# refresh-bio/colord

Hardware: AMD Instinct MI355X
Metric: input Gbases/s + archive size vs ref, ONT 50 Gb at 1/2/4/8 MI355X (higher is better)
Workload: dtype u64

## Files before the change

### colord_amd/csrc/anchors.hip

```cpp
#include "common.hpp"
#include "objects.hpp"
#include <algorithm>

struct cl_anchors {
	cl_ctx* ctx = nullptr;
	uint32_t n_reads = 0, c = 0;
	uint64_t n_anchors = 0;
	DevBuf<uint32_t> n_cands;
	DevBuf<uint32_t> cand;
	DevBuf<uint64_t> cand_off;
	DevBuf<uint32_t> anchors;
};

namespace {

struct Arena { const uint64_t* packed; const uint64_t* word_off; const uint32_t* lens; };

__device__ inline uint64_t mmer_at(const Arena& A, uint64_t wb, uint32_t p, uint32_t m)
{
	const uint64_t* w = A.packed + wb + (p >> 5);
	const uint32_t j = p & 31;
	const uint64_t hi = w[0], lo = w[1];
	const uint32_t s = 128 - 2 * (j + m);
	const uint64_t v = (s >= 64) ? (hi >> (s - 64)) : ((hi << (64 - s)) | (lo >> s));
	return v & ((1ULL << (2 * m)) - 1);
}
__device__ inline uint64_t mmer_of(uint64_t hi, uint64_t lo, uint32_t p, uint32_t m)
{
	const uint32_t s = 128 - 2 * ((p & 31) + m);
	const uint64_t v = (s >= 64) ? (hi >> (s - 64)) : ((hi << (64 - s)) | (lo >> s));
	return v & ((1ULL << (2 * m)) - 1);
}
__device__ inline uint64_t revcomp_m(uint64_t x, uint32_t m)
{
	x = ~x; x = __brevll(x);
	x = ((x >> 1) & 0x5555555555555555ULL) | ((x & 0x5555555555555555ULL) << 1);
	return x >> (64 - 2 * m);
}
__device__ inline uint64_t ref_mmer(const Arena& R, uint32_t id, bool rev, uint32_t q, uint32_t m)
{
	const uint32_t len = R.lens[id];
	const uint64_t wb = R.word_off[id];
	return rev ? revcomp_m(mmer_at(R, wb, len - m - q, m), m) : mmer_at(R, wb, q, m);
}

struct BuildSlot { uint64_t key; uint32_t head; uint32_t strands; };
typedef uint2 EncSlot;
constexpr uint32_t LINK_POS = 0x3fffffffu;
__device__ inline uint32_t tag_of(uint64_t hash) { return (uint32_t)((hash * 0xD6E8FEB86659FD93ULL) >> 32); }
__device__ inline uint32_t table_slot(uint64_t hash, uint32_t tsz) { return (uint32_t)(((uint64_t)(uint32_t)(hash >> 17) * tsz) >> 32); }
struct EncTable { EncSlot* slots; const uint64_t* toff; uint32_t* next; const uint64_t* noff; };
constexpr uint32_t REGION_SLOTS = 2048;
constexpr uint64_t KEY_EMPTY = ~0ULL;
constexpr uint32_t NIL = 0xffffffffu;

__global__ void k_table_sizes(const uint32_t* __restrict__ lens, const uint8_t* __restrict__ has_n, const uint32_t* __restrict__ ncand,
                              uint32_t r0, uint32_t r1, uint32_t m, uint32_t x4, uint32_t lds_max_n, uint32_t* __restrict__ tsize, uint32_t* __restrict__ nsize, uint32_t* __restrict__ err)
{
	uint32_t r = r0 + blockIdx.x * blockDim.x + threadIdx.x;
	if (r >= r1) return;
	uint32_t len = lens[r];
	bool active = ncand[r] > 0 && !has_n[r] && len >= m;
	uint32_t n = active ? len - m + 1 : 0;
	if (n <= lds_max_n) n = 0;
	uint32_t t = 0;
	if (n) { t = 16; while (t < 2 * n + n / 2 && t < REGION_SLOTS) t <<= 1; if (t >= REGION_SLOTS) t = (uint32_t)(((uint64_t)n * x4 / 4 + REGION_SLOTS - 1) / REGION_SLOTS * REGION_SLOTS); }
	tsize[r - r0] = t; nsize[r - r0] = n;
}
constexpr uint32_t REGION = REGION_SLOTS, INS_T = 256;
__global__ __launch_bounds__(INS_T) void k_table_insert(Arena A, uint32_t r0, uint32_t r1, uint32_t m, EncTable T, uint32_t* __restrict__ n_distinct,
                                                       uint2* __restrict__ bins , uint32_t* __restrict__ err)
{
	__shared__ BuildSlot reg[REGION];
	__shared__ uint32_t cnt[512], start[513];
	const uint32_t r = r0 + blockIdx.x;
	if (r >= r1) return;
	const uint64_t t0 = T.toff[r - r0]; const uint32_t tsz = (uint32_t)(T.toff[r - r0 + 1] - t0);
	if (!tsz) return;
	const uint64_t n0 = T.noff[r - r0]; const uint32_t n = (uint32_t)(T.noff[r - r0 + 1] - n0);
	const uint64_t wb = A.word_off[r];
	const uint32_t lane = threadIdx.x & 63;
	const uint32_t rs = tsz < REGION ? tsz : REGION, n_reg = tsz / rs, rshift = 31 - (uint32_t)__clz((int)rs);
	uint2* bin = bins + n0;
	uint32_t fresh = 0;
	for (uint32_t rg0 = 0; rg0 < n_reg; rg0 += 512)
	{
		const uint32_t nr = n_reg - rg0 < 512 ? n_reg - rg0 : 512;
		for (uint32_t i = threadIdx.x; i < 512; i += INS_T) cnt[i] = 0;
		__syncthreads();
		for (uint32_t p = threadIdx.x; p < n; p += INS_T)
		{
			const uint64_t xf = mmer_at(A, wb, p, m), xr = revcomp_m(xf, m), x = xf < xr ? xf : xr;
			const uint32_t h = table_slot(hash_mm(x), tsz), rg = (h >> rshift) - rg0;
			if (rg < nr) atomicAdd(&cnt[rg], 1u);
		}
		__syncthreads();
		if (threadIdx.x == 0) { uint32_t a = 0; for (uint32_t i = 0; i < nr; ++i) { start[i] = a; a += cnt[i]; cnt[i] = 0; } start[nr] = a; }
		__syncthreads();
		for (uint32_t p = threadIdx.x; p < n; p += INS_T)
		{
			const uint64_t xf = mmer_at(A, wb, p, m), xr = revcomp_m(xf, m), x = xf < xr ? xf : xr;
			const uint32_t h = table_slot(hash_mm(x), tsz), rg = (h >> rshift) - rg0;
			if (rg < nr) bin[start[rg] + atomicAdd(&cnt[rg], 1u)] = make_uint2(p, h);
		}
		__syncthreads();
		__threadfence_block();
		for (uint32_t rg = 0; rg < nr; ++rg)
		{
			for (uint32_t i = threadIdx.x; i < rs; i += INS_T) { reg[i].key = KEY_EMPTY; reg[i].head = NIL; reg[i].strands = 0; }
			__syncthreads();
			const uint32_t b = start[rg], e = start[rg + 1];
			for (uint32_t i = b + threadIdx.x; i < e; i += INS_T)
			{
				const uint2 ph = bin[i];
				const uint32_t pp = ph.x;
				const uint64_t xf = mmer_at(A, wb, pp, m), xr = revcomp_m(xf, m), x = xf < xr ? xf : xr;
				uint32_t off = ph.y & (rs - 1), tries = 0;
				for (;;)
				{
					unsigned long long old = atomicCAS((unsigned long long*)&reg[off].key, (unsigned long long)KEY_EMPTY, (unsigned long long)x);
					if (old == KEY_EMPTY || old == x) break;
					off = (off + 1) & (rs - 1);
					if (++tries > rs) { atomicOr(err, 2u); break; }
				}
				const uint32_t strand = xf != x ? 1u : 0u;
				T.next[n0 + pp] = atomicExch(&reg[off].head, pp | (strand << 31));
				if (!(atomicOr(&reg[off].strands, 1u << strand) & (1u << strand))) ++fresh;
			}
			__syncthreads();
			EncSlot* dst = T.slots + t0 + (uint64_t)(rg0 + rg) * rs;
			for (uint32_t i = threadIdx.x; i < rs; i += INS_T) dst[i] = make_uint2(reg[i].head == NIL ? 0u : tag_of(hash_mm(reg[i].key)), reg[i].head);
			__syncthreads();
		}
	}
	fresh = wave_sum(fresh);
	if (lane == 0 && fresh) atomicAdd(&n_distinct[r - r0], fresh);
}
struct TaskCfg { uint32_t r0, r1, c, m; uint32_t pe, pr; double frac_always, frac_min, max_mult; };

constexpr uint32_t FILT_WORDS = 2048, STAGE = 128;
__device__ inline uint32_t filt_word(uint64_t hash) { return (uint32_t)(hash >> 46) & (FILT_WORDS - 1); }
__device__ inline uint64_t filt_mask(uint64_t hash) { return (1ull << ((hash >> 40) & 63)) | (1ull << ((hash >> 34) & 63)) | (1ull << ((hash >> 28) & 63)); }
__device__ __host__ inline uint32_t match_segments(uint32_t n, uint32_t seg_n) { return (seg_n == 0 || n <= seg_n + seg_n / 2) ? 1u : (n + seg_n - 1) / seg_n; }
__global__ __launch_bounds__(256) void k_match(Arena A, Arena R, EncTable T, TaskCfg cfg, const uint32_t* __restrict__ cand_refs, const uint32_t* __restrict__ cand_n,
                                              const uint32_t* __restrict__ n_distinct, const uint2* __restrict__ work , uint32_t n_work, uint32_t seg_n,
                                              unsigned long long* __restrict__ n_pairs, uint64_t cap, uint64_t* __restrict__ pairs)
{
	__shared__ unsigned long long filt[FILT_WORDS];
	__shared__ uint64_t stage_all[4][STAGE];
	if (blockIdx.x >= n_work) return;
	const uint32_t rl = work[blockIdx.x].x, seg = work[blockIdx.x].y;
	const uint32_t lane = threadIdx.x & 63, wv = threadIdx.x >> 6;
	const uint32_t r = cfg.r0 + rl;
	const uint64_t t0 = T.toff[rl]; const uint32_t tsz = (uint32_t)(T.toff[rl + 1] - t0);
	const uint32_t n_slots = cand_n[r] < cfg.c ? cand_n[r] : cfg.c;
	if (tsz == 0 || n_slots == 0) return;
	const uint32_t elen = A.lens[r];
	if ((double)n_distinct[rl] < cfg.frac_min * (double)elen && !((double)n_distinct[rl] > cfg.frac_always * (double)elen)) return;
	for (uint32_t i = threadIdx.x; i < FILT_WORDS; i += 256) filt[i] = 0;
	__syncthreads();
	uint32_t p_lo, p_hi;
	{
		const uint64_t ewb = A.word_off[r]; const uint32_t n = elen - cfg.m + 1;
		const uint32_t nseg = match_segments(n, seg_n);
		if (seg >= nseg) return;
		p_lo = (uint32_t)((uint64_t)n * seg / nseg); p_hi = (uint32_t)((uint64_t)n * (seg + 1) / nseg);
		for (uint32_t p = p_lo + threadIdx.x; p < p_hi; p += 256)
		{
			const uint64_t xf = mmer_at(A, ewb, p, cfg.m), xr = revcomp_m(xf, cfg.m);
			const uint64_t hash = hash_mm(xf < xr ? xf : xr);
			atomicOr(&filt[filt_word(hash)], (unsigned long long)filt_mask(hash));
		}
	}
	__syncthreads();
	const uint64_t n0 = T.noff[rl];
	const uint64_t ewb = A.word_off[r];
	uint64_t* stage = stage_all[wv]; uint32_t fill = 0;
	auto flush = [&]() {
		if (!fill) return;
		unsigned long long base = 0;
		if (lane == 0) base = atomicAdd(n_pairs, (unsigned long long)fill);
		base = ((unsigned long long)__shfl((int)(base >> 32), 0, 64) << 32) | (uint32_t)__shfl((int)(uint32_t)base, 0, 64);
		if (base + fill <= cap) for (uint32_t i = lane; i < fill; i += 64) pairs[base + i] = stage[i];
		fill = 0;
	};
	for (uint32_t slot = 0; slot < n_slots; ++slot)
	{
		const uint32_t id = cand_refs[(uint64_t)r * cfg.c + slot], rlen = R.lens[id];
		if (rlen < cfg.m) continue;
		const uint64_t rwb = R.word_off[id];
		const uint32_t nq = rlen - cfg.m + 1, sl = rl * cfg.c + slot;
		const uint32_t PR = cfg.pr; const uint32_t pr_mask = (1u << PR) - 1;
		const uint64_t key_rev = (uint64_t)(2 * sl) << (cfg.pe + PR), key_fwd = (uint64_t)(2 * sl + 1) << (cfg.pe + PR);
		if (threadIdx.x == 0 && seg == 0) atomicAdd(n_pairs + 1, (unsigned long long)nq);
		const uint64_t* rw = R.packed + rwb;
		struct Probe { uint64_t x; uint2 slot; uint32_t h, tag; bool pass, fwd_other, rev_other; };
		auto probe = [&](uint32_t q, uint64_t hi, uint64_t lo) -> Probe
		{
			Probe P{ 0, make_uint2(0u, NIL), 0, 0, false, false, false };
			if (q < nq)
			{
				const uint64_t y = mmer_of(hi, lo, q, cfg.m), z = revcomp_m(y, cfg.m), x = y < z ? y : z;
				const uint64_t hash = hash_mm(x);
				const uint64_t fm = filt_mask(hash);
				if ((filt[filt_word(hash)] & fm) == fm)
				{
					P.pass = true; P.x = x; P.fwd_other = y != x; P.rev_other = z != x;
					P.h = table_slot(hash, tsz); P.tag = tag_of(hash);
					P.slot = T.slots[t0 + P.h];
				}
			}
			return P;
		};
		uint64_t hi1 = 0, lo1 = 0, hi2 = 0, lo2 = 0;
		Probe cur;
		{
			const uint32_t q = wv * 64 + lane;
			uint64_t hi = 0, lo = 0;
			if (q < nq) { hi = rw[q >> 5]; lo = rw[(q >> 5) + 1]; }
			if (q + 256 < nq) { hi1 = rw[(q + 256) >> 5]; lo1 = rw[((q + 256) >> 5) + 1]; }
			cur = probe(q, hi, lo);
		}
		const uint32_t rmask = (tsz < REGION ? tsz : REGION) - 1;
		for (uint32_t q0 = wv * 64; q0 < nq; q0 += 256)
		{
			const uint32_t q = q0 + lane;
			hi2 = 0; lo2 = 0;
			if (q + 512 < nq) { hi2 = rw[(q + 512) >> 5]; lo2 = rw[((q + 512) >> 5) + 1]; }
			const Probe nxt = probe(q + 256, hi1, lo1);
			uint32_t head = NIL, cnt = 0;
			const uint32_t fs = cur.fwd_other ? 1u : 0u, rs_ = cur.rev_other ? 1u : 0u;
			if (cur.pass)
			{
				uint2 sl8 = cur.slot; uint32_t h = cur.h;
				while (sl8.y != NIL)
				{
					if (sl8.x == cur.tag)
					{
						const uint64_t xf = mmer_at(A, ewb, sl8.y & LINK_POS, cfg.m), xr = revcomp_m(xf, cfg.m);
						if ((xf < xr ? xf : xr) == cur.x) { head = sl8.y; break; }
					}
					h = (h & ~rmask) | ((h + 1) & rmask);
					sl8 = T.slots[t0 + h];
				}
				for (uint32_t p = head; p != NIL; p = T.next[n0 + (p & LINK_POS)])
					if ((p & LINK_POS) >= p_lo && (p & LINK_POS) < p_hi) cnt += (uint32_t)((p >> 31) == fs) + (uint32_t)((p >> 31) == rs_);
			}
			cur = nxt; hi1 = hi2; lo1 = lo2;
			if (!__any(cnt != 0)) continue;
			const uint32_t incl = wave_incl_scan(cnt), tot = __shfl(incl, 63, 64);
			const uint64_t kf = key_fwd | (uint64_t)(~q & pr_mask), kr = key_rev | (uint64_t)(~(nq - 1 - q) & pr_mask);
			if (fill + tot > STAGE) flush();
			if (tot <= STAGE)
			{
				uint32_t o = fill + incl - cnt;
				for (uint32_t p = head; p != NIL; p = T.next[n0 + (p & LINK_POS)])
				{
					if ((p & LINK_POS) < p_lo || (p & LINK_POS) >= p_hi) continue;
					const uint64_t pos = (uint64_t)(p & LINK_POS) << PR;
					if ((p >> 31) == fs) stage[o++] = kf | pos;
					if ((p >> 31) == rs_) stage[o++] = kr | pos;
				}
				fill += tot;
				continue;
			}
			unsigned long long base = 0;
			if (lane == 0) base = atomicAdd(n_pairs, (unsigned long long)tot);
			base = ((unsigned long long)__shfl((int)(base >> 32), 0, 64) << 32) | (uint32_t)__shfl((int)(uint32_t)base, 0, 64);
			if (base + tot > cap) continue;
			uint64_t o = base + incl - cnt;
			for (uint32_t p = head; p != NIL; p = T.next[n0 + (p & LINK_POS)])
			{
				if ((p & LINK_POS) < p_lo || (p & LINK_POS) >= p_hi) continue;
				const uint64_t pos = (uint64_t)(p & LINK_POS) << PR;
				if ((p >> 31) == fs) pairs[o++] = kf | pos;
				if ((p >> 31) == rs_) pairs[o++] = kr | pos;
			}
		}
	}
	flush();
}
template<uint32_t MAXN> struct LdsGeom { static constexpr uint32_t SLOTS = ((MAXN + MAXN / 2) + 17) & ~1u, WORDS = (MAXN + 27 + 31) / 32 + 2; };
__device__ inline uint32_t lds_table_slots(uint32_t n) { const uint32_t s = (n + n / 2 + 1) & ~1u; return s < 16 ? 16 : s; }
template<uint32_t MAXN, uint32_t FW, uint32_t NT, uint32_t WAVES_PER_SIMD>
__global__ __launch_bounds__(NT, WAVES_PER_SIMD) void k_match_lds(Arena A, Arena R, TaskCfg cfg, uint32_t min_n, const uint8_t* __restrict__ has_n,
                                                 const uint32_t* __restrict__ cand_refs, const uint32_t* __restrict__ cand_n, uint32_t* __restrict__ n_distinct, uint32_t n_reads,
                                                 unsigned long long* __restrict__ n_pairs, uint64_t cap, uint64_t* __restrict__ pairs, uint32_t dbg)
{
	static_assert(MAXN <= 65535 && (FW & (FW - 1)) == 0 && NT % 64 == 0, "positions are 16-bit links; 0xffff is the empty slot");
	constexpr uint32_t NW = NT / 64, LSTAGE = 64;
	__shared__ unsigned long long filt[FW];
	__shared__ uint64_t rd[LdsGeom<MAXN>::WORDS];
	__shared__ uint32_t slots32[LdsGeom<MAXN>::SLOTS / 2];
	__shared__ uint64_t stage_all[NW][LSTAGE];
	__shared__ uint32_t s_distinct;
	const uint32_t rl = blockIdx.x;
	if (rl >= n_reads) return;
	const uint32_t r = cfg.r0 + rl, m = cfg.m;
	const uint32_t elen = A.lens[r];
	const uint32_t n_slots = cand_n[r] < cfg.c ? cand_n[r] : cfg.c;
	if (n_slots == 0 || has_n[r] || elen < m) return;
	const uint32_t n = elen - m + 1;
	if (n <= min_n || n > MAXN) return;
	const uint32_t lane = threadIdx.x & 63, wv = threadIdx.x >> 6;
	const uint32_t S = lds_table_slots(n);
	const uint16_t* slot16 = (const uint16_t*)slots32;
	{
		const uint64_t* src = A.packed + A.word_off[r];
		const uint32_t nw = (elen + 31) / 32 + 1;
		for (uint32_t i = threadIdx.x; i < nw; i += NT) rd[i] = src[i];
		for (uint32_t i = threadIdx.x; i < FW; i += NT) filt[i] = 0;
		for (uint32_t i = threadIdx.x; i < S / 2; i += NT) slots32[i] = 0xffffffffu;
		if (threadIdx.x == 0) s_distinct = 0;
	}
	__syncthreads();
	if (dbg == 1) return;
	auto own = [&](uint32_t p) -> uint64_t { return mmer_of(rd[p >> 5], rd[(p >> 5) + 1], p, m); };
	auto step = [&](uint32_t off) -> uint32_t { return off + 1 == S ? 0u : off + 1; };
	{
		uint32_t fresh = 0;
		for (uint32_t p = threadIdx.x; p < n; p += NT)
		{
			const uint64_t xf = own(p), xr = revcomp_m(xf, m), hash = hash_mm(xf < xr ? xf : xr);
			atomicOr(&filt[(uint32_t)(hash >> 46) & (FW - 1)], (unsigned long long)filt_mask(hash));
			bool dup = false;
			for (uint32_t off = table_slot(hash, S);;)
			{
				uint32_t* w = &slots32[off >> 1]; const uint32_t sh = (off & 1) * 16;
				const uint32_t old = *(volatile uint32_t*)w, q = (old >> sh) & 0xffffu;
				if (q != 0xffffu) { if (!dup && own(q) == xf) dup = true; off = step(off); continue; }
				if (atomicCAS(w, old, (old & ~(0xffffu << sh)) | (p << sh)) == old) break;
			}
			fresh += dup ? 0u : 1u;
		}
		fresh = wave_sum(fresh);
		if (lane == 0 && fresh) atomicAdd(&s_distinct, fresh);
	}
	__syncthreads();
	const uint32_t nd = s_distinct;
	if (threadIdx.x == 0) n_distinct[rl] = nd;
	if (dbg == 2) return;
	if ((double)nd < cfg.frac_min * (double)elen && !((double)nd > cfg.frac_always * (double)elen)) return;
	uint64_t* stage = stage_all[wv]; uint32_t fill = 0;
	auto flush = [&]() {
		if (!fill) return;
		unsigned long long base = 0;
		if (lane == 0) base = atomicAdd(n_pairs, (unsigned long long)fill);
		base = ((unsigned long long)__shfl((int)(base >> 32), 0, 64) << 32) | (uint32_t)__shfl((int)(uint32_t)base, 0, 64);
		if (base + fill <= cap) for (uint32_t i = lane; i < fill; i += 64) pairs[base + i] = stage[i];
		fill = 0;
	};
	struct Look { uint64_t y, z; uint32_t h0, cnt, nh, hp0, hp1, hf0, hf1; };
	auto look = [&](bool live, uint32_t q, uint64_t hi, uint64_t lo) -> Look {
		Look L{ 0, 0, 0, 0, 0, 0, 0, 0, 0 };
		if (!live) return L;
// ... 372 lines not shown
		if (i < n)
		{
			const uint32_t t = sel_task[i] & 0x7fffffffu, slot = (t / 2) % c;
			o_cand[4 * s] = cand_refs[(uint64_t)r * c + slot]; o_cand[4 * s + 1] = (t & 1) == 0 ? 1u : 0u;
			o_cand[4 * s + 2] = sel_tot[i]; o_cand[4 * s + 3] = sel_n[i];
			o_task[(uint64_t)rl * c + i] = sel_task[i]; o_count[(uint64_t)rl * c + i] = sel_n[i];
		}
		else { o_cand[4 * s] = ~0u; o_cand[4 * s + 1] = 0; o_cand[4 * s + 2] = 0; o_cand[4 * s + 3] = 0; o_task[(uint64_t)rl * c + i] = ~0u; o_count[(uint64_t)rl * c + i] = 0; }
	}
}
__global__ void k_copy_fix(const uint32_t* __restrict__ o_task, const uint64_t* __restrict__ slot_off, uint64_t n_slots,
                           const uint64_t* __restrict__ pair_off, const uint32_t* __restrict__ anch, uint64_t dst_base, uint32_t* __restrict__ out,
                           TaskCfg cfg, const uint32_t* __restrict__ kanch, const uint64_t* __restrict__ common_off, uint64_t common_base)
{
	const uint64_t s = (uint64_t)blockIdx.x * blockDim.x + threadIdx.x;
	if (s >= n_slots) return;
	const uint32_t tm = o_task[s];
	if (tm == ~0u) return;
	const uint32_t t = tm & 0x7fffffffu;
	const uint32_t n = (uint32_t)(slot_off[s + 1] - slot_off[s]);
	const uint32_t* src = anch + 3 * pair_off[t];
	if (tm & 0x80000000u)
	{
		const uint64_t gs = (uint64_t)cfg.r0 * cfg.c + t / 2;
		const uint64_t o = common_off[gs] - common_base; const uint32_t nk = (uint32_t)(common_off[gs + 1] - common_off[gs]);
		src = kanch + 6 * o + (uint64_t)(t & 1) * 3 * nk;
	}
	uint32_t* dst = out + 3 * (dst_base + slot_off[s]);
	for (uint32_t i = 0; i < 3 * n; ++i) dst[i] = src[i];
	for (uint32_t i = 0; i + 1 < n; ++i)
	{
		const uint32_t end = dst[3 * i + 2] + dst[3 * i];
		if (dst[3 * (i + 1) + 2] < end) { const uint32_t d = end - dst[3 * (i + 1) + 2]; dst[3 * (i + 1) + 2] += d; dst[3 * (i + 1)] -= d; dst[3 * (i + 1) + 1] += d; }
	}
	for (uint32_t i = 0; i + 1 < n; ++i)
	{
		const uint32_t end = dst[3 * i + 1] + dst[3 * i];
		if (dst[3 * (i + 1) + 1] < end) { const uint32_t d = end - dst[3 * (i + 1) + 1]; dst[3 * (i + 1) + 1] += d; dst[3 * (i + 1)] -= d; dst[3 * (i + 1) + 2] += d; }
	}
}
__global__ void k_add_u64(uint64_t* v, uint64_t n, uint64_t c) { uint64_t i = (uint64_t)blockIdx.x * blockDim.x + threadIdx.x; if (i < n) v[i] += c; }
}

extern "C" cl_status cl_anchor_candidates_hifi(cl_ctx* ctx, const cl_reads* reads, const cl_reads* refs, const uint32_t* d_cand_refs, const uint32_t* d_cand_n,
                                               uint32_t c, uint32_t anchor_len, double frac_always, double frac_min, double max_matches_mult,
                                               uint32_t min_anchors, uint32_t kmer_len, uint32_t modulo, const uint64_t* d_common_off, const uint64_t* d_common, cl_anchors** out);
extern "C" cl_status cl_anchor_candidates(cl_ctx* ctx, const cl_reads* reads, const cl_reads* refs, const uint32_t* d_cand_refs, const uint32_t* d_cand_n,
                                          uint32_t c, uint32_t anchor_len, double frac_always, double frac_min, double max_matches_mult,
                                          uint32_t min_anchors, cl_anchors** out)
{
	return cl_anchor_candidates_hifi(ctx, reads, refs, d_cand_refs, d_cand_n, c, anchor_len, frac_always, frac_min, max_matches_mult, min_anchors, 0, 0, nullptr, nullptr, out);
}
extern "C" cl_status cl_anchor_candidates_hifi(cl_ctx* ctx, const cl_reads* reads, const cl_reads* refs, const uint32_t* d_cand_refs, const uint32_t* d_cand_n,
                                               uint32_t c, uint32_t anchor_len, double frac_always, double frac_min, double max_matches_mult,
                                               uint32_t min_anchors, uint32_t kmer_len, uint32_t modulo, const uint64_t* d_common_off, const uint64_t* d_common, cl_anchors** out)
{
	if (!ctx || !reads || !refs || !d_cand_refs || !d_cand_n || !out) return cl_fail(ctx, CL_E_INVALID, "cl_anchor_candidates: null argument");
	const bool hifi = d_common_off != nullptr;
	if (hifi && (kmer_len < 2 || kmer_len > 28 || modulo == 0)) return cl_fail(ctx, CL_E_INVALID, "cl_anchor_candidates_hifi: 2 <= kmer_len <= 28, modulo >= 1");
	if (c == 0 || c > 16 || anchor_len < 2 || anchor_len > 28) return cl_fail(ctx, CL_E_INVALID, "cl_anchor_candidates: 1 <= c <= 16, 2 <= anchor_len <= 28");
	HIP_TRY(ctx, hipSetDevice(ctx->device));
	const uint32_t nr = reads->n_reads, m = anchor_len;
	cl_anchors* X = new cl_anchors(); X->ctx = ctx; X->n_reads = nr; X->c = c;
	std::unique_ptr<cl_anchors> guard(X);
	DEV_ALLOC(ctx, X->n_cands, nr); DEV_ALLOC(ctx, X->cand, (uint64_t)nr * c * 4); DEV_ALLOC(ctx, X->cand_off, (uint64_t)nr * c + 1);
	Arena A{ reads->packed.p, reads->word_off.p, reads->lens.p }, R{ refs->packed.p, refs->word_off.p, refs->lens.p };
	std::vector<uint32_t> h_len(nr);
	if (nr) HIP_TRY(ctx, hipMemcpy(h_len.data(), reads->lens.p, (uint64_t)nr * 4, hipMemcpyDeviceToHost));
	auto bits_for = [](uint64_t v) -> uint32_t { uint32_t b = 1; while ((1ull << b) <= v) ++b; return b; };
	uint32_t max_ref_len = 0;
	if (refs->n_reads)
	{
		std::vector<uint32_t> rl(refs->n_reads);
		HIP_TRY(ctx, hipMemcpy(rl.data(), refs->lens.p, (uint64_t)refs->n_reads * 4, hipMemcpyDeviceToHost));
		for (uint32_t l : rl) max_ref_len = std::max(max_ref_len, l);
	}
	const uint32_t pr_bits = bits_for(max_ref_len);
	const uint64_t BATCH_BASES = 1ull << 28;
	std::vector<DevBuf<uint32_t>> chunks; std::vector<uint64_t> chunk_n;
	uint64_t total_anchors = 0;
	double pairs_per_base = 0.5;
	struct TableBatch {
		uint32_t r0 = 0, r1 = 0, pe = 1; uint64_t acc = 0, nsum = 0;
		DevBuf<uint32_t> n_distinct, next, err; DevBuf<uint64_t> toff, noff; DevBuf<EncSlot> slots; DevBuf<uint2> bins;
		std::vector<uint2> h_work; DevBuf<uint2> work;
		struct SideSync { hipStream_t s = nullptr; ~SideSync() { if (s) (void)hipStreamSynchronize(s); } } sync;
	};
	HIP_TRY(ctx, cl_side_stream(ctx, ctx->side));
	constexpr uint32_t LDS_N_A = 12288, LDS_N_B = 24576, LDS_NT = 1024;
	uint32_t lds_max_n = 0;
	if (const char* e = getenv("COLORD_HIP_ANCHORS_LDS")) lds_max_n = atoi(e) <= 0 ? 0u : (uint32_t)atoi(e) <= LDS_N_A ? LDS_N_A : LDS_N_B;
	const uint32_t match_seg = getenv("COLORD_HIP_MATCH_SEG") ? (uint32_t)std::max(0, atoi(getenv("COLORD_HIP_MATCH_SEG"))) : 16384u;
	const uint32_t lds_dbg = getenv("COLORD_HIP_LDS_DBG") ? (uint32_t)atoi(getenv("COLORD_HIP_LDS_DBG")) : 0u;
	auto prepare = [&](uint32_t r0, std::unique_ptr<TableBatch>& out) -> cl_status {
		out = std::make_unique<TableBatch>();
		TableBatch& B = *out;
		uint32_t r1 = r0; uint64_t acc = 0;
		uint32_t mx = 0;
		while (r1 < nr && (r1 == r0 || acc + h_len[r1] <= BATCH_BASES))
		{
			const uint32_t pe = bits_for(std::max(mx, h_len[r1]));
			if (r1 > r0 && pe + pr_bits + bits_for((r1 - r0 + 1) * 2 * c) > 64) break;
			mx = std::max(mx, h_len[r1]); acc += h_len[r1]; ++r1;
		}
		B.r0 = r0; B.r1 = r1; B.acc = acc; B.pe = bits_for(mx);
		for (uint32_t r = r0; r < r1; ++r)
			for (uint32_t sg = 0, ns = match_segments(h_len[r] >= m ? h_len[r] - m + 1 : 0, match_seg); sg < ns; ++sg) B.h_work.push_back(make_uint2(r - r0, sg));
		if (B.pe + pr_bits + bits_for((r1 - r0) * 2 * c) > 64) return cl_fail(ctx, CL_E_UNSUPPORTED, "cl_anchor_candidates: a read and its candidates are too long for 64-bit match keys");
		const uint32_t nb = r1 - r0;
		const uint32_t table_x4 = 8;
		LaunchOn on(ctx, ctx->side);
		B.sync.s = ctx->side;
		DevBuf<uint32_t> tsize, nsize, err; DEV_ALLOC(ctx, tsize, nb); DEV_ALLOC(ctx, nsize, nb); DEV_ALLOC(ctx, err, 1); DEV_ALLOC(ctx, B.n_distinct, nb);
		HIP_TRY(ctx, hipMemsetAsync(err.p, 0, 4, ctx->side));
		LAUNCH(ctx, k_table_sizes, grid_for(nb, 256), 256, (const uint32_t*)reads->lens.p, (const uint8_t*)reads->has_n.p, d_cand_n, r0, r1, m, table_x4, lds_max_n, tsize.p, nsize.p, err.p);
		DEV_ALLOC(ctx, B.toff, (uint64_t)nb + 1); DEV_ALLOC(ctx, B.noff, (uint64_t)nb + 1);
		uint64_t tsum = 0;
		CL_TRY(dev_exclusive_scan_u64(ctx, tsize.p, B.toff.p, nb, &tsum));
		CL_TRY(dev_exclusive_scan_u64(ctx, nsize.p, B.noff.p, nb, &B.nsum));
		uint32_t herr = 0; HIP_TRY(ctx, hipMemcpyAsync(&herr, err.p, 4, hipMemcpyDeviceToHost, ctx->side)); HIP_TRY(ctx, hipStreamSynchronize(ctx->side));
		DEV_ALLOC(ctx, B.slots, tsum); DEV_ALLOC(ctx, B.next, B.nsum); DEV_ALLOC(ctx, B.bins, B.nsum); DEV_ALLOC(ctx, B.err, 1);
		DEV_ALLOC(ctx, B.work, B.h_work.size() + 1);
		if (!B.h_work.empty()) HIP_TRY(ctx, hipMemcpyAsync(B.work.p, B.h_work.data(), B.h_work.size() * sizeof(uint2), hipMemcpyHostToDevice, ctx->side));
		HIP_TRY(ctx, hipMemsetAsync(B.n_distinct.p, 0, (uint64_t)nb * 4, ctx->side));
		HIP_TRY(ctx, hipMemsetAsync(B.err.p, 0, 4, ctx->side));
		EncTable T{ B.slots.p, B.toff.p, B.next.p, B.noff.p };
		LAUNCHB(ctx, B.nsum * (0.25 + 16.0) , k_table_insert, nb, INS_T, A, r0, r1, m, T, B.n_distinct.p, B.bins.p, B.err.p);
		HIP_TRY(ctx, hipGetLastError());
		return CL_OK;
	};
	std::unique_ptr<TableBatch> cur, nxt;
	if (nr) CL_TRY(prepare(0, cur));
	while (cur)
	{
		const uint32_t r0 = cur->r0, r1 = cur->r1; const uint64_t acc = cur->acc;
		const uint32_t nb = r1 - r0, n_tasks = nb * 2 * c;
		TaskCfg cfg{ r0, r1, c, m, cur->pe, pr_bits, frac_always, frac_min, max_matches_mult };
		HIP_TRY(ctx, hipStreamSynchronize(ctx->stream));
		HIP_TRY(ctx, hipStreamSynchronize(ctx->side));
		cur->sync.s = nullptr;
		{ uint32_t herr = 0; HIP_TRY(ctx, hipMemcpy(&herr, cur->err.p, 4, hipMemcpyDeviceToHost)); if (herr) return cl_fail(ctx, CL_E_UNSUPPORTED, "cl_anchor_candidates: a region of an m-mer table overflowed"); }
		DevBuf<uint32_t>& n_distinct = cur->n_distinct;
		EncTable T{ cur->slots.p, cur->toff.p, cur->next.p, cur->noff.p };
		DevBuf<uint32_t> pair_cnt; DEV_ALLOC(ctx, pair_cnt, (uint64_t)n_tasks + 1);
		DevBuf<uint64_t> pair_off; DEV_ALLOC(ctx, pair_off, (uint64_t)n_tasks + 1);
		DevBuf<unsigned long long> d_np; DEV_ALLOC(ctx, d_np, 4);
		DevBuf<uint64_t> pairs;
		uint64_t n_pairs = 0;
		for (uint64_t cap = (uint64_t)(pairs_per_base * 1.25 * (double)acc) + (1u << 20);;)
		{
			DEV_ALLOC(ctx, pairs, cap);
			HIP_TRY(ctx, hipMemsetAsync(d_np.p, 0, 32, ctx->stream));
			if (lds_max_n)
			{
				LAUNCH_NAMED(ctx, "k_match_lds<12288>", (k_match_lds<LDS_N_A, 2048, LDS_NT, 8>), nb, LDS_NT, A, R, cfg, 0u, (const uint8_t*)reads->has_n.p, d_cand_refs, d_cand_n, n_distinct.p, nb, d_np.p, cap, pairs.p, lds_dbg);
				if (lds_max_n > LDS_N_A)
					LAUNCH_NAMED(ctx, "k_match_lds<24576>", (k_match_lds<LDS_N_B, 4096, LDS_NT, 4>), nb, LDS_NT, A, R, cfg, LDS_N_A, (const uint8_t*)reads->has_n.p, d_cand_refs, d_cand_n, n_distinct.p, nb, d_np.p, cap, pairs.p, lds_dbg);
			}
			LAUNCHB(ctx, 0.0, k_match, (uint32_t)cur->h_work.size(), 256, A, R, T, cfg, d_cand_refs, d_cand_n, (const uint32_t*)n_distinct.p, (const uint2*)cur->work.p, (uint32_t)cur->h_work.size(), match_seg, d_np.p, cap, pairs.p);
			HIP_TRY(ctx, hipGetLastError());
			unsigned long long h_np2[2] = { 0, 0 };
			HIP_TRY(ctx, hipMemcpyAsync(h_np2, d_np.p, 16, hipMemcpyDeviceToHost, ctx->stream));
			if (r1 < nr && !nxt) CL_TRY(prepare(r1, nxt));
			HIP_TRY(ctx, hipStreamSynchronize(ctx->stream));
			const unsigned long long h_np = h_np2[0];
			n_pairs = h_np;
			if (ctx->timing && !ctx->pending_bytes.empty()) ctx->pending_bytes.back() = (double)h_np2[1] * 8.25 + (double)std::min<uint64_t>(h_np, cap) * 8.0;
			if (getenv("COLORD_HIP_ANCHOR_DEBUG")) fprintf(stderr, "[anchors] batch reads %u..%u bases %llu: pairs %llu cap %llu\n", r0, r1, (unsigned long long)acc, h_np, (unsigned long long)cap);
			if (n_pairs >= (1ull << 32)) return cl_fail(ctx, CL_E_UNSUPPORTED, "cl_anchor_candidates: batch produces >= 2^32 match pairs");
			if (n_pairs <= cap) break;
			cap = n_pairs;
		}
		if (acc) pairs_per_base = std::max(pairs_per_base, (double)n_pairs / (double)acc);
		DevBuf<int> tf, ts, pred; DEV_ALLOC(ctx, tf, n_pairs); DEV_ALLOC(ctx, ts, n_pairs); DEV_ALLOC(ctx, pred, n_pairs);
		DevBuf<uint32_t> anch; DEV_ALLOC(ctx, anch, 3 * n_pairs);
		DevBuf<uint32_t> t_nanch, t_tot; DEV_ALLOC(ctx, t_nanch, n_tasks); DEV_ALLOC(ctx, t_tot, n_tasks);
		if (n_pairs)
		{
			uint32_t tb = 1; while ((1ull << tb) < n_tasks) ++tb;
			CL_TRY(dev_sort_pairs(ctx, pairs.p, nullptr, n_pairs, 0, cfg.pe + cfg.pr + tb));
		}
		LAUNCH(ctx, k_task_pairs, grid_for((uint64_t)n_tasks + 1, 256), 256, (const uint64_t*)pairs.p, n_pairs, A, cfg, (const uint32_t*)n_distinct.p, n_tasks, pair_off.p, pair_cnt.p);
		LAUNCHB(ctx, n_pairs * 32.0, k_lis_anchors, grid_for(n_tasks, 64), 64, A, R, cfg, d_cand_refs, n_tasks, (const uint64_t*)pair_off.p, (const uint32_t*)pair_cnt.p, (const uint64_t*)pairs.p,
			tf.p, ts.p, pred.p, anch.p, t_nanch.p, t_tot.p, (uint32_t)(getenv("COLORD_HIP_LIS_DBG") ? atoi(getenv("COLORD_HIP_LIS_DBG")) : 0));
		HIP_TRY(ctx, hipGetLastError());
		const uint64_t n_slots = (uint64_t)nb * c;
		DevBuf<uint64_t> k_sorted; DevBuf<uint32_t> k_tab, kanch, k_n, k_tot; DevBuf<uint8_t> k_use;
		uint64_t common_base = 0;
		if (hifi)
		{
			uint64_t hb[2] = { 0, 0 };
			HIP_TRY(ctx, hipMemcpy(&hb[0], d_common_off + (uint64_t)r0 * c, 8, hipMemcpyDeviceToHost));
			HIP_TRY(ctx, hipMemcpy(&hb[1], d_common_off + (uint64_t)r1 * c, 8, hipMemcpyDeviceToHost));
			common_base = hb[0];
			const uint64_t nk = hb[1] - hb[0];
			DEV_ALLOC(ctx, k_sorted, nk + 1); DEV_ALLOC(ctx, k_tab, 8 * nk + 8); DEV_ALLOC(ctx, kanch, 6 * nk + 6);
			DEV_ALLOC(ctx, k_n, 2 * n_slots); DEV_ALLOC(ctx, k_tot, 2 * n_slots); DEV_ALLOC(ctx, k_use, n_slots);
			KmerArgs ka{ d_common, d_common_off, k_sorted.p, k_tab.p, kanch.p, k_n.p, k_tot.p, k_use.p, common_base, kmer_len, make_modtest(modulo) };
			LAUNCH(ctx, k_kmer_anchors, grid_for(n_slots, 64), 64, A, R, cfg, d_cand_refs, d_cand_n, (const uint8_t*)reads->has_n.p, (const uint32_t*)n_distinct.p, ka);
			HIP_TRY(ctx, hipGetLastError());
		}
		DevBuf<uint32_t> o_task, o_count; DEV_ALLOC(ctx, o_task, n_slots); DEV_ALLOC(ctx, o_count, n_slots);
		LAUNCH(ctx, k_select, grid_for(nb, 128), 128, cfg, d_cand_refs, d_cand_n, min_anchors, (const uint32_t*)t_nanch.p, (const uint32_t*)t_tot.p,
			(const uint8_t*)(hifi ? k_use.p : nullptr), (const uint32_t*)k_n.p, (const uint32_t*)k_tot.p,
			X->n_cands.p, X->cand.p, o_task.p, o_count.p);
		DevBuf<uint64_t> slot_off; DEV_ALLOC(ctx, slot_off, n_slots + 1);
		uint64_t n_here = 0;
		CL_TRY(dev_exclusive_scan_u64(ctx, o_count.p, slot_off.p, n_slots, &n_here));
		DevBuf<uint32_t> chunk; DEV_ALLOC(ctx, chunk, 3 * n_here);
		LAUNCH(ctx, k_copy_fix, grid_for(n_slots, 128), 128, (const uint32_t*)o_task.p, (const uint64_t*)slot_off.p, n_slots, (const uint64_t*)pair_off.p,
			(const uint32_t*)anch.p, (uint64_t)0, chunk.p, cfg, (const uint32_t*)kanch.p, d_common_off, common_base);
		HIP_TRY(ctx, hipMemcpyAsync(X->cand_off.p + (uint64_t)r0 * c, slot_off.p, n_slots * 8, hipMemcpyDeviceToDevice, ctx->stream));
		if (total_anchors) LAUNCH(ctx, k_add_u64, grid_for(n_slots, 256), 256, X->cand_off.p + (uint64_t)r0 * c, n_slots, total_anchors);
		HIP_TRY(ctx, hipGetLastError());
		HIP_TRY(ctx, hipStreamSynchronize(ctx->stream));
		chunks.push_back(std::move(chunk)); chunk_n.push_back(n_here);
		total_anchors += n_here;
		cur = std::move(nxt);
	}
	X->n_anchors = total_anchors;
	DEV_ALLOC(ctx, X->anchors, 3 * total_anchors);
	uint64_t o = 0;
	for (size_t i = 0; i < chunks.size(); ++i)
	{
		if (chunk_n[i]) HIP_TRY(ctx, hipMemcpyAsync(X->anchors.p + 3 * o, chunks[i].p, chunk_n[i] * 12, hipMemcpyDeviceToDevice, ctx->stream));
		o += chunk_n[i];
	}
	HIP_TRY(ctx, hipMemcpyAsync(X->cand_off.p + (uint64_t)nr * c, &total_anchors, 8, hipMemcpyHostToDevice, ctx->stream));
	HIP_TRY(ctx, hipStreamSynchronize(ctx->stream));
	cl_timing_collect(ctx);
	*out = guard.release();
	return CL_OK;
}
extern "C" void cl_anchors_free(cl_anchors* a) { delete a; }
extern "C" uint64_t cl_anchors_total(const cl_anchors* a) { return a->n_anchors; }
extern "C" const uint32_t* cl_anchors_n_cands(const cl_anchors* a) { return a->n_cands.p; }
extern "C" const uint32_t* cl_anchors_cands(const cl_anchors* a) { return a->cand.p; }
extern "C" const uint64_t* cl_anchors_cand_offsets(const cl_anchors* a) { return a->cand_off.p; }
extern "C" const uint32_t* cl_anchors_data(const cl_anchors* a) { return a->anchors.p; }
```

Baseline: 2.959.

## Store table chains as region-ordered link pairs and tile the m-mer binning

The m-mer table build now bins positions through a shared-memory tile with block-wide scans, writing them grouped by region into a combined link array of (position, next-index) pairs. This replaces the separate bins and next arrays and the serial thread-0 prefix sum. It also skips binning entirely when a read has a single region, and batches the fill loop so each thread handles four entries with the loads hoisted ahead. The match kernel walks chains through the new link array, so each hop reads one 8-byte entry whose next index points into region-local storage, aiming for better locality than scattered per-position next lookups. It costs extra shared-memory phases and syncs per tile and a more complex indexing scheme; the host-side sync ordering is also adjusted for error handling.

Result: no change. 2.978, median of 3 (+0.6%).

```diff
diff --git a/colord_amd/csrc/anchors.hip b/colord_amd/csrc/anchors.hip
--- a/colord_amd/csrc/anchors.hip
+++ b/colord_amd/csrc/anchors.hip
@@ -49,7 +49,7 @@
 constexpr uint32_t LINK_POS = 0x3fffffffu;
 __device__ inline uint32_t tag_of(uint64_t hash) { return (uint32_t)((hash * 0xD6E8FEB86659FD93ULL) >> 32); }
 __device__ inline uint32_t table_slot(uint64_t hash, uint32_t tsz) { return (uint32_t)(((uint64_t)(uint32_t)(hash >> 17) * tsz) >> 32); }
-struct EncTable { EncSlot* slots; const uint64_t* toff; uint32_t* next; const uint64_t* noff; };
+struct EncTable { EncSlot* slots; const uint64_t* toff; uint2* links; const uint64_t* noff; };
 constexpr uint32_t REGION_SLOTS = 2048;
 constexpr uint64_t KEY_EMPTY = ~0ULL;
 constexpr uint32_t NIL = 0xffffffffu;
@@ -67,71 +67,162 @@
 	if (n) { t = 16; while (t < 2 * n + n / 2 && t < REGION_SLOTS) t <<= 1; if (t >= REGION_SLOTS) t = (uint32_t)(((uint64_t)n * x4 / 4 + REGION_SLOTS - 1) / REGION_SLOTS * REGION_SLOTS); }
 	tsize[r - r0] = t; nsize[r - r0] = n;
 }
-constexpr uint32_t REGION = REGION_SLOTS, INS_T = 256;
-__global__ __launch_bounds__(INS_T) void k_table_insert(Arena A, uint32_t r0, uint32_t r1, uint32_t m, EncTable T, uint32_t* __restrict__ n_distinct,
-                                                       uint2* __restrict__ bins , uint32_t* __restrict__ err)
-{
-	__shared__ BuildSlot reg[REGION];
-	__shared__ uint32_t cnt[512], start[513];
+constexpr uint32_t REGION = REGION_SLOTS, INS_T = 256, BIN_TILE = 4096, BIN_PER_T = BIN_TILE / INS_T, FILL_PER_T = 4, MAX_REG = 512;
+__global__ __launch_bounds__(INS_T) void k_table_insert(Arena A, uint32_t r0, uint32_t r1, uint32_t m, EncTable T, uint32_t* __restrict__ n_distinct, uint32_t* __restrict__ err)
+{
+	__shared__ __attribute__((aligned(16))) unsigned char smem[REGION * sizeof(BuildSlot)];
+	__shared__ uint32_t cnt[MAX_REG], start[MAX_REG + 1];
+	BuildSlot* reg = (BuildSlot*)smem;
+	uint32_t* tile_x = (uint32_t*)smem;
+	uint16_t* tile_rg = (uint16_t*)(smem + BIN_TILE * 4);
+	uint32_t* tcnt = (uint32_t*)(smem + BIN_TILE * 6);
+	uint32_t* tstart = tcnt + MAX_REG;
+	uint32_t* wsum = tstart + MAX_REG;
+	static_assert(BIN_TILE * 6 + MAX_REG * 8 + 16 <= REGION * sizeof(BuildSlot), "the tile and its counters live in the region array");
+	static_assert(INS_T == 256 && MAX_REG == 2 * INS_T, "the scans below take two regions a thread, four waves");
 	const uint32_t r = r0 + blockIdx.x;
 	if (r >= r1) return;
 	const uint64_t t0 = T.toff[r - r0]; const uint32_t tsz = (uint32_t)(T.toff[r - r0 + 1] - t0);
 	if (!tsz) return;
 	const uint64_t n0 = T.noff[r - r0]; const uint32_t n = (uint32_t)(T.noff[r - r0 + 1] - n0);
 	const uint64_t wb = A.word_off[r];
-	const uint32_t lane = threadIdx.x & 63;
+	const uint32_t lane = threadIdx.x & 63, wv = threadIdx.x >> 6;
 	const uint32_t rs = tsz < REGION ? tsz : REGION, n_reg = tsz / rs, rshift = 31 - (uint32_t)__clz((int)rs);
-	uint2* bin = bins + n0;
+	uint2* lk = T.links + n0;
+	const uint64_t* rw = A.packed + wb;
+	static_assert(32 % BIN_PER_T == 0 && BIN_PER_T + 28 + (32 - BIN_PER_T) <= 64, "a thread's positions of a tile share two words");
 	uint32_t fresh = 0;
-	for (uint32_t rg0 = 0; rg0 < n_reg; rg0 += 512)
-	{
-		const uint32_t nr = n_reg - rg0 < 512 ? n_reg - rg0 : 512;
-		for (uint32_t i = threadIdx.x; i < 512; i += INS_T) cnt[i] = 0;
+	auto scan2 = [&](uint32_t a0, uint32_t a1, uint32_t& e0, uint32_t& e1) -> uint32_t {
+		const uint32_t s2 = a0 + a1, incl = wave_incl_scan(s2);
 		__syncthreads();
-		for (uint32_t p = threadIdx.x; p < n; p += INS_T)
-		{
-			const uint64_t xf = mmer_at(A, wb, p, m), xr = revcomp_m(xf, m), x = xf < xr ? xf : xr;
-			const uint32_t h = table_slot(hash_mm(x), tsz), rg = (h >> rshift) - rg0;
-			if (rg < nr) atomicAdd(&cnt[rg], 1u);
-		}
+		if (lane == 63) wsum[wv] = incl;
 		__syncthreads();
-		if (threadIdx.x == 0) { uint32_t a = 0; for (uint32_t i = 0; i < nr; ++i) { start[i] = a; a += cnt[i]; cnt[i] = 0; } start[nr] = a; }
+		uint32_t before = 0, total = 0;
+		for (uint32_t w = 0; w < INS_T / 64; ++w) { const uint32_t x = wsum[w]; total += x; if (w < wv) before += x; }
+		e0 = before + incl - s2; e1 = e0 + a0;
+		return total;
+	};
+	uint32_t rbase = 0;
+	for (uint32_t rg0 = 0; rg0 < n_reg; rg0 += MAX_REG)
+	{
+		const uint32_t nr = n_reg - rg0 < MAX_REG ? n_reg - rg0 : MAX_REG;
+		if (n_reg == 1)
+		{
+			if (threadIdx.x == 0) { start[0] = 0; start[1] = n; }
+			__syncthreads();
+		}
+		else
+		{
+			for (uint32_t i = threadIdx.x; i < MAX_REG; i += INS_T) cnt[i] = 0;
+			__syncthreads();
+			for (uint32_t tb = 0; tb < n; tb += BIN_TILE)
+			{
+				const uint32_t p0 = tb + threadIdx.x * BIN_PER_T;
+				if (p0 >= n) continue;
+				const uint64_t hi = rw[p0 >> 5], lo = rw[(p0 >> 5) + 1];
+#pragma unroll
+				for (uint32_t j = 0; j < BIN_PER_T; ++j)
+				{
+					const uint32_t p = p0 + j;
+					if (p >= n) break;
+					const uint64_t xf = mmer_of(hi, lo, p, m), xr = revcomp_m(xf, m), x = xf < xr ? xf : xr;
+					const uint32_t h = table_slot(hash_mm(x), tsz), rg = (h >> rshift) - rg0;
+					if (rg < nr) atomicAdd(&cnt[rg], 1u);
+				}
+			}
+			__syncthreads();
+			{
+				const uint32_t a0 = cnt[2 * threadIdx.x], a1 = cnt[2 * threadIdx.x + 1];
+				uint32_t e0, e1;
+				const uint32_t total = scan2(a0, a1, e0, e1);
+				start[2 * threadIdx.x] = e0; start[2 * threadIdx.x + 1] = e1;
+				if (threadIdx.x == INS_T - 1) start[MAX_REG] = total;
+				cnt[2 * threadIdx.x] = 0; cnt[2 * threadIdx.x + 1] = 0;
+			}
+			__syncthreads();
+			for (uint32_t tb = 0; tb < n; tb += BIN_TILE)
+			{
+				tcnt[2 * threadIdx.x] = 0; tcnt[2 * threadIdx.x + 1] = 0;
+				__syncthreads();
+				uint32_t kx[BIN_PER_T], kr[BIN_PER_T];
+				const uint32_t p0 = tb + threadIdx.x * BIN_PER_T;
+				uint64_t hi = 0, lo = 0;
+				if (p0 < n) { hi = rw[p0 >> 5]; lo = rw[(p0 >> 5) + 1]; }
+#pragma unroll
+				for (uint32_t j = 0; j < BIN_PER_T; ++j)
+				{
+					const uint32_t p = p0 + j;
+					kx[j] = 0; kr[j] = NIL;
+					if (p < n)
+					{
+						const uint64_t xf = mmer_of(hi, lo, p, m), xr = revcomp_m(xf, m), x = xf < xr ? xf : xr;
+						const uint32_t h = table_slot(hash_mm(x), tsz), rg = (h >> rshift) - rg0;
+						if (rg < nr) { kx[j] = p | (xf != x ? 0x80000000u : 0u); kr[j] = rg | (atomicAdd(&tcnt[rg], 1u) << 9); }
+					}
+				}
+				__syncthreads();
+				uint32_t in_tile;
+				{
+					const uint32_t a0 = tcnt[2 * threadIdx.x], a1 = tcnt[2 * threadIdx.x + 1];
+					uint32_t e0, e1;
+					in_tile = scan2(a0, a1, e0, e1);
+					tstart[2 * threadIdx.x] = e0; tstart[2 * threadIdx.x + 1] = e1;
+					tcnt[2 * threadIdx.x] = start[2 * threadIdx.x] + cnt[2 * threadIdx.x] - e0; tcnt[2 * threadIdx.x + 1] = start[2 * threadIdx.x + 1] + cnt[2 * threadIdx.x + 1] - e1;
+					cnt[2 * threadIdx.x] += a0; cnt[2 * threadIdx.x + 1] += a1;
+				}
+				__syncthreads();
+#pragma unroll
+				for (uint32_t j = 0; j < BIN_PER_T; ++j)
+					if (kr[j] != NIL) { const uint32_t rg = kr[j] & (MAX_REG - 1), at = tstart[rg] + (kr[j] >> 9); tile_x[at] = kx[j]; tile_rg[at] = (uint16_t)rg; }
+				__syncthreads();
+				for (uint32_t j = threadIdx.x; j < in_tile; j += INS_T) lk[rbase + j + tcnt[tile_rg[j]]] = make_uint2(tile_x[j], NIL);
+				__syncthreads();
+			}
+			__threadfence_block();
+		}
+		for (uint32_t i = threadIdx.x; i < rs; i += INS_T) { reg[i].key = KEY_EMPTY; reg[i].head = NIL; reg[i].strands = 0; }
 		__syncthreads();
-		for (uint32_t p = threadIdx.x; p < n; p += INS_T)
-		{
-			const uint64_t xf = mmer_at(A, wb, p, m), xr = revcomp_m(xf, m), x = xf < xr ? xf : xr;
-			const uint32_t h = table_slot(hash_mm(x), tsz), rg = (h >> rshift) - rg0;
-			if (rg < nr) bin[start[rg] + atomicAdd(&cnt[rg], 1u)] = make_uint2(p, h);
-		}
-		__syncthreads();
-		__threadfence_block();
 		for (uint32_t rg = 0; rg < nr; ++rg)
 		{
-			for (uint32_t i = threadIdx.x; i < rs; i += INS_T) { reg[i].key = KEY_EMPTY; reg[i].head = NIL; reg[i].strands = 0; }
-			__syncthreads();
-			const uint32_t b = start[rg], e = start[rg + 1];
-			for (uint32_t i = b + threadIdx.x; i < e; i += INS_T)
-			{
-				const uint2 ph = bin[i];
-				const uint32_t pp = ph.x;
-				const uint64_t xf = mmer_at(A, wb, pp, m), xr = revcomp_m(xf, m), x = xf < xr ? xf : xr;
-				uint32_t off = ph.y & (rs - 1), tries = 0;
-				for (;;)
+			const uint32_t b = rbase + start[rg], e = rbase + start[rg + 1];
+			for (uint32_t i0 = b + threadIdx.x; i0 < e; i0 += FILL_PER_T * INS_T)
+			{
+				uint32_t pp[FILL_PER_T]; uint64_t hi[FILL_PER_T], lo[FILL_PER_T];
+#pragma unroll
+				for (uint32_t k = 0; k < FILL_PER_T; ++k) { const uint32_t i = i0 + k * INS_T; pp[k] = i >= e ? NIL : n_reg == 1 ? i : lk[i].x & LINK_POS; }
+#pragma unroll
+				for (uint32_t k = 0; k < FILL_PER_T; ++k) { hi[k] = 0; lo[k] = 0; if (pp[k] != NIL) { hi[k] = rw[pp[k] >> 5]; lo[k] = rw[(pp[k] >> 5) + 1]; } }
+#pragma unroll
+				for (uint32_t k = 0; k < FILL_PER_T; ++k)
 				{
-					unsigned long long old = atomicCAS((unsigned long long*)&reg[off].key, (unsigned long long)KEY_EMPTY, (unsigned long long)x);
-					if (old == KEY_EMPTY || old == x) break;
-					off = (off + 1) & (rs - 1);
-					if (++tries > rs) { atomicOr(err, 2u); break; }
+					if (pp[k] == NIL) continue;
+					const uint32_t i = i0 + k * INS_T;
+					const uint64_t xf = mmer_of(hi[k], lo[k], pp[k], m), xr = revcomp_m(xf, m), x = xf < xr ? xf : xr;
+					uint32_t off = table_slot(hash_mm(x), tsz) & (rs - 1), tries = 0;
+					for (;;)
+					{
+						unsigned long long old = atomicCAS((unsigned long long*)&reg[off].key, (unsigned long long)KEY_EMPTY, (unsigned long long)x);
+						if (old == KEY_EMPTY || old == x) break;
+						off = (off + 1) & (rs - 1);
+						if (++tries > rs) { atomicOr(err, 2u); break; }
+					}
+					const uint32_t strand = xf != x ? 1u : 0u;
+					lk[i] = make_uint2(pp[k] | (strand << 31), atomicExch(&reg[off].head, i));
+					if (!(atomicOr(&reg[off].strands, 1u << strand) & (1u << strand))) ++fresh;
 				}
-				const uint32_t strand = xf != x ? 1u : 0u;
-				T.next[n0 + pp] = atomicExch(&reg[off].head, pp | (strand << 31));
-				if (!(atomicOr(&reg[off].strands, 1u << strand) & (1u << strand))) ++fresh;
 			}
 			__syncthreads();
 			EncSlot* dst = T.slots + t0 + (uint64_t)(rg0 + rg) * rs;
-			for (uint32_t i = threadIdx.x; i < rs; i += INS_T) dst[i] = make_uint2(reg[i].head == NIL ? 0u : tag_of(hash_mm(reg[i].key)), reg[i].head);
+			for (uint32_t i = threadIdx.x; i < rs; i += INS_T)
+			{
+				const uint32_t head = reg[i].head;
+				dst[i] = make_uint2(head == NIL ? 0u : tag_of(hash_mm(reg[i].key)), head);
+				reg[i].key = KEY_EMPTY; reg[i].head = NIL; reg[i].strands = 0;
+			}
 			__syncthreads();
 		}
+		rbase += start[nr];
+		__syncthreads();
 	}
 	fresh = wave_sum(fresh);
 	if (lane == 0 && fresh) atomicAdd(&n_distinct[r - r0], fresh);
@@ -173,7 +264,7 @@
 		}
 	}
 	__syncthreads();
-	const uint64_t n0 = T.noff[rl];
+	const uint2* L = T.links + T.noff[rl];
 	const uint64_t ewb = A.word_off[r];
 	uint64_t* stage = stage_all[wv]; uint32_t fill = 0;
 	auto flush = [&]() {
@@ -237,14 +328,17 @@
 				{
 					if (sl8.x == cur.tag)
 					{
-						const uint64_t xf = mmer_at(A, ewb, sl8.y & LINK_POS, cfg.m), xr = revcomp_m(xf, cfg.m);
+						const uint64_t xf = mmer_at(A, ewb, L[sl8.y].x & LINK_POS, cfg.m), xr = revcomp_m(xf, cfg.m);
 						if ((xf < xr ? xf : xr) == cur.x) { head = sl8.y; break; }
 					}
 					h = (h & ~rmask) | ((h + 1) & rmask);
 					sl8 = T.slots[t0 + h];
 				}
-				for (uint32_t p = head; p != NIL; p = T.next[n0 + (p & LINK_POS)])
+				for (uint32_t i = head; i != NIL;)
+				{
+					const uint2 e = L[i]; const uint32_t p = e.x; i = e.y;
 					if ((p & LINK_POS) >= p_lo && (p & LINK_POS) < p_hi) cnt += (uint32_t)((p >> 31) == fs) + (uint32_t)((p >> 31) == rs_);
+				}
 			}
 			cur = nxt; hi1 = hi2; lo1 = lo2;
 			if (!__any(cnt != 0)) continue;
@@ -254,8 +348,9 @@
 			if (tot <= STAGE)
 			{
 				uint32_t o = fill + incl - cnt;
-				for (uint32_t p = head; p != NIL; p = T.next[n0 + (p & LINK_POS)])
+				for (uint32_t i = head; i != NIL;)
 				{
+					const uint2 e = L[i]; const uint32_t p = e.x; i = e.y;
 					if ((p & LINK_POS) < p_lo || (p & LINK_POS) >= p_hi) continue;
 					const uint64_t pos = (uint64_t)(p & LINK_POS) << PR;
 					if ((p >> 31) == fs) stage[o++] = kf | pos;
@@ -269,8 +364,9 @@
 			base = ((unsigned long long)__shfl((int)(base >> 32), 0, 64) << 32) | (uint32_t)__shfl((int)(uint32_t)base, 0, 64);
 			if (base + tot > cap) continue;
 			uint64_t o = base + incl - cnt;
-			for (uint32_t p = head; p != NIL; p = T.next[n0 + (p & LINK_POS)])
-			{
+			for (uint32_t i = head; i != NIL;)
+			{
+				const uint2 e = L[i]; const uint32_t p = e.x; i = e.y;
 				if ((p & LINK_POS) < p_lo || (p & LINK_POS) >= p_hi) continue;
 				const uint64_t pos = (uint64_t)(p & LINK_POS) << PR;
 				if ((p >> 31) == fs) pairs[o++] = kf | pos;
@@ -809,7 +905,7 @@
 	double pairs_per_base = 0.5;
 	struct TableBatch {
 		uint32_t r0 = 0, r1 = 0, pe = 1; uint64_t acc = 0, nsum = 0;
-		DevBuf<uint32_t> n_distinct, next, err; DevBuf<uint64_t> toff, noff; DevBuf<EncSlot> slots; DevBuf<uint2> bins;
+		DevBuf<uint32_t> n_distinct, err; DevBuf<uint64_t> toff, noff; DevBuf<EncSlot> slots; DevBuf<uint2> links;
 		std::vector<uint2> h_work; DevBuf<uint2> work;
 		struct SideSync { hipStream_t s = nullptr; ~SideSync() { if (s) (void)hipStreamSynchronize(s); } } sync;
 	};
@@ -846,13 +942,14 @@
 		CL_TRY(dev_exclusive_scan_u64(ctx, tsize.p, B.toff.p, nb, &tsum));
 		CL_TRY(dev_exclusive_scan_u64(ctx, nsize.p, B.noff.p, nb, &B.nsum));
 		uint32_t herr = 0; HIP_TRY(ctx, hipMemcpyAsync(&herr, err.p, 4, hipMemcpyDeviceToHost, ctx->side)); HIP_TRY(ctx, hipStreamSynchronize(ctx->side));
-		DEV_ALLOC(ctx, B.slots, tsum); DEV_ALLOC(ctx, B.next, B.nsum); DEV_ALLOC(ctx, B.bins, B.nsum); DEV_ALLOC(ctx, B.err, 1);
+		DEV_ALLOC(ctx, B.slots, tsum); DEV_ALLOC(ctx, B.links, B.nsum); DEV_ALLOC(ctx, B.err, 1);
 		DEV_ALLOC(ctx, B.work, B.h_work.size() + 1);
 		if (!B.h_work.empty()) HIP_TRY(ctx, hipMemcpyAsync(B.work.p, B.h_work.data(), B.h_work.size() * sizeof(uint2), hipMemcpyHostToDevice, ctx->side));
 		HIP_TRY(ctx, hipMemsetAsync(B.n_distinct.p, 0, (uint64_t)nb * 4, ctx->side));
 		HIP_TRY(ctx, hipMemsetAsync(B.err.p, 0, 4, ctx->side));
-		EncTable T{ B.slots.p, B.toff.p, B.next.p, B.noff.p };
-		LAUNCHB(ctx, B.nsum * (0.25 + 16.0) , k_table_insert, nb, INS_T, A, r0, r1, m, T, B.n_distinct.p, B.bins.p, B.err.p);
+		EncTable T{ B.slots.p, B.toff.p, B.links.p, B.noff.p };
+		LAUNCHB(ctx, B.nsum * (0.25 + 16.0 + 8.0 + 8.0) ,
+			k_table_insert, nb, INS_T, A, r0, r1, m, T, B.n_distinct.p, B.err.p);
 		HIP_TRY(ctx, hipGetLastError());
 		return CL_OK;
 	};
@@ -868,7 +965,7 @@
 		cur->sync.s = nullptr;
 		{ uint32_t herr = 0; HIP_TRY(ctx, hipMemcpy(&herr, cur->err.p, 4, hipMemcpyDeviceToHost)); if (herr) return cl_fail(ctx, CL_E_UNSUPPORTED, "cl_anchor_candidates: a region of an m-mer table overflowed"); }
 		DevBuf<uint32_t>& n_distinct = cur->n_distinct;
-		EncTable T{ cur->slots.p, cur->toff.p, cur->next.p, cur->noff.p };
+		EncTable T{ cur->slots.p, cur->toff.p, cur->links.p, cur->noff.p };
 		DevBuf<uint32_t> pair_cnt; DEV_ALLOC(ctx, pair_cnt, (uint64_t)n_tasks + 1);
 		DevBuf<uint64_t> pair_off; DEV_ALLOC(ctx, pair_off, (uint64_t)n_tasks + 1);
 		DevBuf<unsigned long long> d_np; DEV_ALLOC(ctx, d_np, 4);
@@ -888,8 +985,10 @@
 			HIP_TRY(ctx, hipGetLastError());
 			unsigned long long h_np2[2] = { 0, 0 };
 			HIP_TRY(ctx, hipMemcpyAsync(h_np2, d_np.p, 16, hipMemcpyDeviceToHost, ctx->stream));
-			if (r1 < nr && !nxt) CL_TRY(prepare(r1, nxt));
-			HIP_TRY(ctx, hipStreamSynchronize(ctx->stream));
+			const cl_status prep = (r1 < nr && !nxt) ? prepare(r1, nxt) : CL_OK;
+			const hipError_t waited = hipStreamSynchronize(ctx->stream);
+			CL_TRY(prep);
+			HIP_TRY(ctx, waited);
 			const unsigned long long h_np = h_np2[0];
 			n_pairs = h_np;
 			if (ctx->timing && !ctx->pending_bytes.empty()) ctx->pending_bytes.back() = (double)h_np2[1] * 8.25 + (double)std::min<uint64_t>(h_np, cap) * 8.0;
```
